# nghiahuynh-ai/Flamed-TTS

Hardware: AMD Instinct MI355X
Metric: latent frames/s (RTF at nsteps-denoiser=128) (higher is better)
Workload: dtype bf16; 1 GPU; BASELINE configs[1]: 1 utterance(s) x 400 frames (5.0 s audio) per GPU, nsteps-denoiser=128, bf16 (one persistent launch per solve); batch_per_gpu=1, frames=400, nfe=128, global_batch=1, parallelism=utterance-sharded x1 (no collectives)

## Files before the change

### flamed-tts_amd/csrc/capi.cpp

```cpp
#include <cstdarg>
#include <cstdio>
#include <cstring>
#include <mutex>

#include "common.hpp"
#include "flamed_hip.h"

namespace fl {
static thread_local char g_err[1024] = "";

void set_error(const char* fmt, ...) {
  va_list ap;
  va_start(ap, fmt);
  vsnprintf(g_err, sizeof(g_err), fmt, ap);
  va_end(ap);
}
const char* last_error() { return g_err; }

int device_of(const void* p, int* dev) {
  if (!p || !dev) return kBadArg;
  hipPointerAttribute_t a;
  if (hipPointerGetAttributes(&a, p) != hipSuccess) {
    (void)hipGetLastError();
    return kBadArg;
// ... 34 lines not shown
  static const int k_smax[] = {1, 2, 4, 0};
  static const Knob knobs[] = {
      {"splitk_target", &Tune::split_target, 1, 1 << 20, nullptr},
      {"splitk_max", &Tune::split_max, 1, 4, k_smax},
      {"small_stages", &Tune::small_stages, 3, 7, k_stages},
      {"xcd_strips", &Tune::xcd_strips, 0, 64, nullptr},
      {"bn32", &Tune::bn32, 0, 1, nullptr},
      {"dma", &Tune::use_dma, 0, 2, nullptr},
      {"dma_ns", &Tune::dma_ns, 3, 8, k_dmans},
      {"noctr", &Tune::noctr, 0, 1, nullptr},
      {"dup_class", &Tune::dup_class, -1, FLAMED_DEN_KERNEL_CLASSES - 1, nullptr},
      {"stamp_class", &Tune::stamp_class, -1, FLAMED_DEN_KERNEL_CLASSES - 1, nullptr},
      {"dw_cg32", &Tune::dw_cg32_rows, 0, 1 << 30, nullptr},
      {"dw_cg", &Tune::dw_cg_small, 16, 32, k_dwcg},
      {"dw_tc", &Tune::dw_tc_big, 64, 128, k_dwtc},
      {"big", &Tune::big, 0, 1, nullptr},
      {"big_rows", &Tune::big_min_rows, 1024, 1 << 30, nullptr},
      {"big_ns", &Tune::big_ns, 2, 3, k_bigns},
      {"lnfold", &Tune::lnfold, 0, 1, nullptr},
      {"fold_rows", &Tune::fold_big_rows, 0, 1 << 30, nullptr},
      {"graph_steps", &Tune::graph_steps, 1, 1024, nullptr},
      {"x16", &Tune::x16, 0, 1, nullptr},
      {"g8p_rows", &Tune::g8p_rows, 0, 1 << 30, nullptr},
      {"dwgn", &Tune::dwgn, 0, 1, nullptr},
      {"dwgn_small", &Tune::dwgn_small, 0, 1, nullptr},
      {"fuse_euler", &Tune::fuse_euler, 0, 1, nullptr},
      {"pva_split", &Tune::pva_split, 0, 1, nullptr},
      {"persist", &Tune::persist, 0, 1, nullptr},
      {"split_batch", &Tune::split_batch, 1, 4, nullptr},
      {"split_graph", &Tune::split_graph, 0, 1, nullptr},
      {"split_prio", &Tune::split_prio, 0, 2, nullptr},
      {"prio_all", &Tune::prio_all, 0, 1, nullptr},
      {"split_min_rows", &Tune::split_min_rows, 1024, 1 << 30, nullptr},
      {"persist_opt", &Tune::persist_opt, 0, (1 << 23) - 1, nullptr},
      {"persist_seal_skip", &Tune::persist_seal_skip, -1, 1 << 20, nullptr},
      {"persist_inject", &Tune::persist_inject, -1, 1 << 20, nullptr},
      {"persist_multi", &Tune::persist_multi, 0, 1, nullptr},
      {"persist_pad", &Tune::persist_pad, 0, 1, nullptr},
      {"persist_pad_ntw", &Tune::persist_pad_ntw, 1, 8, nullptr},
      {"persist_as", &Tune::persist_as, 0, 8, nullptr},
      {"persist_multi_ntw", &Tune::persist_multi_ntw, 1, 8, nullptr},
      {"persist_ntw", &Tune::persist_ntw, 1, 8, nullptr},
      {"persist_capmode", &Tune::persist_capmode, 0, 1, nullptr},
      {"pva_persist", &Tune::pva_persist, 0, 1, nullptr},
      {"attn_mfma", &Tune::attn_mfma, 0, 1, nullptr},
      {"prior_split", &Tune::prior_split, 0, 1, nullptr},
      {"enc_skip", &Tune::enc_skip, 0, 1, nullptr},
      {"stop_after", &Tune::stop_after, -1, 1 << 20, nullptr},
      {"coop", &Tune::coop, 0, 1, nullptr},
      {"dwgn_var", &Tune::dwgn_var, 0, 2, nullptr},
      {"pva_stage", &Tune::pva_stage, 0, 3, nullptr},
      {"pva_inject", &Tune::pva_inject, -1, 1 << 20, nullptr},
      {"adaln_grouped", &Tune::adaln_grouped, 0, 1, nullptr},
  };
  for (const Knob& k : knobs) {
    if (std::strcmp(k.name, key) != 0) continue;
    int v = value;
    if (k.lo == 0 && k.hi == 1) v = value != 0;
    FL_REQUIRE(v >= k.lo && v <= k.hi, "flamed_tune: %s must be in [%d, %d] (got %d)", key, k.lo, k.hi, value);
    if (k.allowed) {
      bool ok = false;
      for (const int* a = k.allowed; *a; ++a) ok = ok || *a == v;
      FL_REQUIRE(ok, "flamed_tune: %s = %d is not a supported value", key, value);
    }
    t.*(k.field) = v;
    return kOk;
  }
// ... 20 lines not shown
```

### flamed-tts_amd/csrc/persist.hip

```cpp
#include <cstdio>
#include <cstdlib>

#include "flamed_hip.h"
#include "flamed_diag.h"
#include "persist.hpp"
#include "gemm_dma.hpp"

namespace fl {
namespace pk {

#ifdef FL_STAMPS
constexpr int kStampSlots = 160;
#define PST(step)                                                                                       \
  do {                                                                                                  \
    if ((step) == P.pst_step && P.pst && threadIdx.x == 0 && pst_k < kStampSlots)                       \
      P.pst[blockIdx.x * kStampSlots + pst_k] = __builtin_amdgcn_s_memrealtime();                      \
    ++pst_k;                                                                                            \
  } while (0)
#define PSTP(step) \
  (((step) == P.pst_step && P.pst && pst_k < kStampSlots) ? P.pst + blockIdx.x * kStampSlots + pst_k++ : (++pst_k, nullptr))
#define GND(k, v)                                                                                       \
  do {                                                                                                  \
    if (cur_step == P.gnd_step && P.gnd)                                                                \
      P.gnd[(((size_t)blk * kWGs + g * kSlots + s) * 32 + (tid & 31)) * 32 + (k)] = (v);                \
// ... 152 lines not shown
}

template <int K, class RowB>
__device__ __forceinline__ void dma_panel4(char* dst, const void* base, RowB rowb, int wave, int lane_in, bool w4 = true) {
  constexpr int kRowB = 2 * K, kNI = 32 * kRowB / 1024;
  static_assert(kNI % 4 == 0, "pieces per wave");
  if (!w4 && wave == 0) return;
  const int w0 = w4 ? wave : wave - 1, ws = w4 ? 4 : 3;
  const int lane = opq(lane_in);
  const unsigned long long b = (unsigned long long)(uintptr_t)base;
  const unsigned blo = (unsigned)__builtin_amdgcn_readfirstlane((unsigned)b);
  const unsigned bhi = (unsigned)__builtin_amdgcn_readfirstlane((unsigned)(b >> 32));
  const unsigned long long bs = ((unsigned long long)bhi << 32) | (unsigned long long)blo;
  const unsigned l0 = __builtin_amdgcn_readfirstlane((unsigned)(uintptr_t)((__attribute__((address_space(3))) char*)(dst)));
#pragma unroll
  for (int j = 0; j < (kNI + 2) / 3; ++j) {
    const int i = w0 + ws * j;
    if (i >= kNI) break;
    const unsigned pos = (unsigned)i * 1024u + (unsigned)lane * 16u;
    const int n = (int)(pos / kRowB);
    const unsigned jl = (pos % kRowB) >> 4;
    const unsigned off = rowb(n) + ((jl ^ (unsigned)(n & 15)) << 4);
    const unsigned l = l0 + (unsigned)i * 1024u;
    unsigned keep;
    asm volatile("s_mov_b32 %0, m0\n\ts_mov_b32 m0, %3\n\ts_nop 0\n\tglobal_load_lds_dwordx4 %1, %2\n\ts_mov_b32 m0, %0"
                 : "=&s"(keep)
                 : "v"(off), "s"(bs), "s"(l)
                 : "memory");
  }
}

__device__ __forceinline__ unsigned frag_group_bytes(int KST) { return (unsigned)(4 * kMaxNTW * KST * 1024); }

template <int K>
__device__ __forceinline__ void gemm(const bf16* A, int r0, int nr, const char* wl, f32x4 (&acc)[2], int wave, int lane_in,
                                     unsigned long long* stamp = nullptr, int g = 0, bool frag = false, int tile = -1,
                                     bool first = true) {
  constexpr int KST = K / 32;
  const int lane = opq(lane_in);
  if (tile < 0) tile = wave;
  acc[0] = f32x4{0.f, 0.f, 0.f, 0.f};
  acc[1] = f32x4{0.f, 0.f, 0.f, 0.f};
  const int ntile = (nr + 15) >> 4;
  const int c = lane & 15, q = lane >> 4;
  u32x4 a[KST];
  if (tile < ntile) {
    if (frag) {
      const __amdgpu_buffer_rsrc_t rs =
          rsrc(reinterpret_cast<const char*>(A) + (size_t)g * frag_group_bytes(KST), frag_group_bytes(KST));
      const unsigned base = (unsigned)(((tile * KST) * 64 + lane) * 16);
#pragma unroll
      for (int ks = 0; ks < KST; ++ks) a[ks] = ld16(rs, base + ks * 1024);
    } else {
      const __amdgpu_buffer_rsrc_t rs = rsrc(A + (size_t)r0 * K, (unsigned)nr * K * 2);
      const unsigned base = (unsigned)(((16 * tile + c) * K + q * 8) * 2);
#pragma unroll
      for (int ks = 0; ks < KST; ++ks) a[ks] = ld16(rs, base + ks * 64);
    }
    if (first) asm volatile("s_waitcnt vmcnt(%0)" ::"i"(KST) : "memory");
    else asm volatile("s_waitcnt vmcnt(0)" ::: "memory");
  } else {
    asm volatile("s_waitcnt vmcnt(0)" ::: "memory");
  }
  if (first) __syncthreads();
  if (first && stamp && threadIdx.x == 0) *stamp = __builtin_amdgcn_s_memrealtime();
  if (tile < ntile) {
    constexpr int kBP = 4;
    u32x4 b0[kBP], b1[kBP];
#pragma unroll
    for (int p = 0; p < kBP; ++p) {
      b0[p] = *reinterpret_cast<const u32x4*>(wl + woff<K>(c, 4 * p + q));
      b1[p] = *reinterpret_cast<const u32x4*>(wl + woff<K>(16 + c, 4 * p + q));
    }
#pragma unroll
    for (int ks = 0; ks < KST; ++ks) {
      const u32x4 x0 = b0[ks % kBP], x1 = b1[ks % kBP];
      if (ks + kBP < KST) {
        b0[ks % kBP] = *reinterpret_cast<const u32x4*>(wl + woff<K>(c, 4 * (ks + kBP) + q));
        b1[ks % kBP] = *reinterpret_cast<const u32x4*>(wl + woff<K>(16 + c, 4 * (ks + kBP) + q));
      }
      acc[0] = __builtin_amdgcn_mfma_f32_16x16x32_bf16(__builtin_bit_cast(bf16x8, x0), __builtin_bit_cast(bf16x8, a[ks]), acc[0], 0, 0, 0);
      acc[1] = __builtin_amdgcn_mfma_f32_16x16x32_bf16(__builtin_bit_cast(bf16x8, x1), __builtin_bit_cast(bf16x8, a[ks]), acc[1], 0, 0, 0);
    }
  }
}

template <int K, int NTW>
__device__ __forceinline__ void gemm_multi(const bf16* A, int r0, int nr, const char* wl, f32x4 (&acc)[NTW][2], int wave,
                                           int lane_in, unsigned long long* stamp, int g, bool frag) {
  constexpr int KST = K / 32, KU = KST / 2, U = 2 * NTW;
  static_assert(KST % 2 == 0, "half-tile units");
  const int lane = opq(lane_in);
  const int ntile = (nr + 15) >> 4;
  const int c = lane & 15, q = lane >> 4;
  const __amdgpu_buffer_rsrc_t rs = frag ? rsrc(reinterpret_cast<const char*>(A) + (size_t)g * frag_group_bytes(KST), frag_group_bytes(KST))
                                         : rsrc(A + (size_t)r0 * K, (unsigned)nr * K * 2);
  u32x4 a[2][KU];
  auto load = [&](u32x4 (&dst)[KU], int u) __attribute__((always_inline)) {
    const int tile = wave + 4 * (u >> 1), k0 = (u & 1) * KU;
    if (tile >= ntile) return;
    if (frag) {
      const unsigned base = (unsigned)(((tile * KST + k0) * 64 + lane) * 16);
#pragma unroll
      for (int ks = 0; ks < KU; ++ks) dst[ks] = ld16(rs, base + ks * 1024);
    } else {
      const unsigned base = (unsigned)(((16 * tile + c) * K + k0 * 32 + q * 8) * 2);
#pragma unroll
      for (int ks = 0; ks < KU; ++ks) dst[ks] = ld16(rs, base + ks * 64);
    }
  };
  load(a[0], 0);
  if (wave < ntile) asm volatile("s_waitcnt vmcnt(%0)" ::"i"(KU) : "memory");
// ... 405 lines not shown

__device__ __forceinline__ float2 gn_finalize(const float (&nv)[kGroups], const float (&mv)[kGroups], const float (&qv)[kGroups],
                                              int utt, int gpu, int T, float gw) {
#pragma clang fp contract(off)
  float n = 0.f, mean = 0.f, m2 = 0.f;
#pragma unroll
  for (int k = 0; k < kGroups; ++k) {
    const bool mine = k / gpu == utt;
    chan_combine_rn(n, mean, m2, mine ? nv[k] : 0.f, mine ? mv[k] : 0.f, mine ? qv[k] : 0.f);
  }
  return make_float2(mean, (1.0f / sqrtf(m2 * (1.0f / (float)T) + 1e-5f)) * gw);
}

template <bool KH, int NTW, bool RK2 = false, bool RAG = false>
__global__ __launch_bounds__(kThreads, 1) void den_persist_kernel(Params P) {
  extern __shared__ __attribute__((aligned(16))) char smem[];
  const int tid = threadIdx.x, lane = tid & 63;
  const int wave = __builtin_amdgcn_readfirstlane(tid >> 6);
  const int T = P.T;
  const int TT = P.B * P.T;
  const int H = kH;
  int g = blockIdx.x % kGroups, s = blockIdx.x / kGroups;
  if (P.opt & 8) {
    const int x = g, j = s;
    g = 4 * (x / 4) + (j % 4);
    s = 8 * (x % 4) + j / 4;
  }
  constexpr bool xloc = false;
  const bool frag = (P.opt & 64) != 0;
  constexpr bool kDefer = NTW == 1 && !KH;
  const bool gran = (P.opt & 512) != 0;
  constexpr bool kTileMajor = true;
  const bool tm = kTileMajor && !(P.opt & 2097152);
  const int gpu = kGroups / P.B, utt = g / gpu;
  auto len_of = [&](int k) {
    if constexpr (RAG) return P.lens[k / gpu];
    else return T;
  };
  const int Tu = len_of(g);
  int r0, nr;
  group_rows(g, T, Tu, P.B, r0, nr, P.opt);
  const int ub = utt * T, ue = ub + Tu;
  const bool idle = P.Bx > 0 && utt >= P.Bx;
  const int MB = P.Bx > 0 ? P.Bx : P.B, mutt = idle ? P.Bx - 1 : utt;
  const int c = lane & 15, q = lane >> 4;
  const int col0 = kCols * s;
  char* stg = smem + L_HS;
  float* hs = reinterpret_cast<float*>(smem + L_HS);
  float* st = reinterpret_cast<float*>(smem + L_ST);
  float* red = reinterpret_cast<float*>(smem + L_RED);
  float4* gnv = reinterpret_cast<float4*>(smem + L_GNV);
  int* flag = reinterpret_cast<int*>(smem + L_FLAG);
  constexpr bool kOneWord = one_word_variant(KH, NTW, RK2, RAG);
  const ArriveImage ai = arrive_image(kOneWord ? kOptOneWord : P.opt, g, s);
  int* const grp = P.ctr + (kOneWord ? CT_GRP : ai.abase());
  int* const mygrp = kOneWord ? grp + 16 * g : P.ctr + ai.base;
  int* const mysig = kOneWord ? mygrp : P.ctr + ai.sig;
  const int gws = kOneWord ? 0 : ai.stride(), gwn = kOneWord ? 1 : ai.n();
  const int aws = kOneWord ? 16 : ai.stride(), awn = kOneWord ? kGroups : ai.an();
  auto gtarget = [&](int l) { return kOneWord ? 32 * l : ai.target(l); };
  int* gnc = P.ctr + CT_GN + 16 * s;
  int* errw = P.ctr + CT_ERR;
  int* fails = P.sticky + SY_FAILS;
  const long long tmo = P.tmo;
  int L = 0;
  int ndg = 0;
// ... 44 lines not shown
  const int xr_row = tid >> 2, xch = kCh * s + 2 * (tid & 3);
  float xs0[NTW], xs1[NTW];
#pragma unroll
  for (int i = 0; i < NTW; ++i) {
    xs0[i] = 0.f;
    xs1[i] = 0.f;
    const int row = kChunk * i + xr_row;
    if (row < nr && !idle) {
      xs0[i] = P.xt[(size_t)(r0 + row) * kC + xch];
      xs1[i] = P.xt[(size_t)(r0 + row) * kC + xch + 1];
    }
  }
  constexpr bool kStash = RK2 && NTW >= 3;
  [[maybe_unused]] float xb0[RK2 && !kStash ? NTW : 1], xb1[RK2 && !kStash ? NTW : 1];
  if constexpr (RK2 && !kStash) {
#pragma unroll
    for (int i = 0; i < NTW; ++i) {
      xb0[i] = xs0[i];
      xb1[i] = xs1[i];
    }
  }
  const bool seal = (P.opt & 16384) != 0;
  const bool dseal = (P.opt & 65536) != 0;
  int dseal_v = 0x7fffffff, dseal_tgt = 0;
  auto dseal_check = [&]() {
    if (dseal && wave == 0) {
      const bool ok = __all(dseal_v >= dseal_tgt);
      if (!ok && lane == 0) raise_err(errw, fails, 4);
      return ok;
    }
    return true;
  };
  auto seal_put = [&]() {
    dseal_check();
    if ((seal || dseal) && tid == 0 && !(cur_step == P.seal_skip && blockIdx.x == 5))
      __hip_atomic_store(P.seal + 4 * (g * kSlots + s), L + 1, __ATOMIC_RELAXED, __HIP_MEMORY_SCOPE_AGENT);
  };
  auto seal_wait = [&](int g0, int ng) -> bool {
    if (dseal) {
      if (wave == 0) {
        const int gi = ng == 1 ? g0 : (lane < 32 ? (g + kGroups - 1) % kGroups : (g + 1) % kGroups);
        dseal_v = __hip_atomic_load(P.seal + 4 * (gi * kSlots + (lane & 31)), __ATOMIC_RELAXED, __HIP_MEMORY_SCOPE_AGENT);
        dseal_tgt = L;
      }
      return true;
    }
    return !seal || seals_ok(P.seal + 4 * g0 * kSlots, ng * kSlots, L, P.ctr + CT_ERR, P.sticky + SY_FAILS, P.tmo,
                             reinterpret_cast<int*>(smem + L_FLAG));
  };
  auto fail_exit = [&]() {
#pragma unroll
    for (int i = 0; i < NTW; ++i) {
      const int row = kChunk * i + xr_row;
      if (row < nr && !idle) {
        P.xt[(size_t)(r0 + row) * kC + xch] = __builtin_nanf("");
        P.xt[(size_t)(r0 + row) * kC + xch + 1] = __builtin_nanf("");
      }
    }
  };
  const bool wlocal = (P.opt & 32768) != 0;
  auto stage_sync = [&]() {
    if (wlocal) asm volatile("s_waitcnt lgkmcnt(0)" ::: "memory");
    else __syncthreads();
  };
  dma_panel<kC>(smem, [&](int n) { return P.win + (size_t)(col0 + n) * kC; }, wave, lane, P.opt);
  auto publish_xs = [&]() {
    bf16* t = reinterpret_cast<bf16*>(stg);
#pragma unroll
    for (int i = 0; i < NTW; ++i) {
      const int nrc = crows(i);
      if (i > 0) stage_sync();
      t[xr_row * kCh + 2 * (tid & 3)] = (bf16)xs0[i];
      t[xr_row * kCh + 2 * (tid & 3) + 1] = (bf16)xs1[i];
      stage_sync();
      const int prow = 16 * wave + lane;
      if (frag) {
        if (lane < 16 && 16 * wave < nrc) {
          const __amdgpu_buffer_rsrc_t rs =
              rsrc(reinterpret_cast<char*>(P.xs) + (size_t)g * frag_group_bytes(kC / 32), frag_group_bytes(kC / 32));
          const int tt = 4 * i + wave, ln = lane + 16 * (s & 3);
          const u32x4 v = prow < nrc ? *reinterpret_cast<const u32x4*>(stg + prow * 16) : u32x4{0u, 0u, 0u, 0u};
          const unsigned off = (unsigned)(((tt * (kC / 32) + (s >> 2)) * 64 + ln) * 16);
          if (xloc) st16p(rs, off, v);
          else st16(rs, off, v);
        }
      } else if (lane < 16 && prow < nrc) {
        const __amdgpu_buffer_rsrc_t rs = rsrc(P.xs, (unsigned)TT * kC * 2);
        const unsigned off = (unsigned)(((size_t)(r0 + kChunk * i + prow) * kC + kCh * s) * 2);
        if (xloc) st16p(rs, off, *reinterpret_cast<const u32x4*>(stg + prow * 16));
        else st16(rs, off, *reinterpret_cast<const u32x4*>(stg + prow * 16));
      }
    }
    seal_put();
    signal(mysig);
    ++L;
  };
  {
    unsigned* const a0 = reinterpret_cast<unsigned*>(P.sticky + SY_ARRIVE0);
    unsigned* const a1 = reinterpret_cast<unsigned*>(P.sticky + SY_ARRIVE1);
    unsigned* tk = reinterpret_cast<unsigned*>(smem + L_FLAG);
    if (tid == 0) tk[1] = __hip_atomic_fetch_add(a0, 1u, __ATOMIC_RELAXED, __HIP_MEMORY_SCOPE_AGENT);
    __syncthreads();
    const unsigned target = arrive_target(tk[1]);
    __syncthreads();
    const bool ok0 = arrive_wait(a0, target, tmo, flag);
    if (ok0) {
      constexpr int kRst = kOneWord ? 4 : kResetInts, kRstN = kOneWord ? kCtrOneInts : kCtrInts;
      if (tid < kRst && kRstN > kRst * (int)blockIdx.x + tid)
        __hip_atomic_store(P.ctr + kRst * blockIdx.x + tid, 0, __ATOMIC_RELAXED, __HIP_MEMORY_SCOPE_AGENT);
      if (tid < 4) __hip_atomic_store(P.seal + 4 * blockIdx.x + tid, 0, __ATOMIC_RELAXED, __HIP_MEMORY_SCOPE_AGENT);
      if (gran && tid < 32) {
        const __amdgpu_buffer_rsrc_t rq = rsrc(P.gnp, kGroups * kH * 16);
        st16(rq, (unsigned)((blockIdx.x * 32 + tid) * 16), u32x4{0u, 0u, 0u, 0u});
      }
      if (tid < 8) {
        const __amdgpu_buffer_rsrc_t ry = rsrc(P.yb, kWGs * 2 * kCh * 8);
        st16(ry, (unsigned)((blockIdx.x * 8 + tid) * 16), u32x4{0u, 0u, 0u, 0u});
      }
      asm volatile("s_waitcnt vmcnt(0)" ::: "memory");
    }
    __syncthreads();
    if (tid == 0) __hip_atomic_fetch_add(a1, 1u, __ATOMIC_RELAXED, __HIP_MEMORY_SCOPE_AGENT);
    const bool ok1 = arrive_wait(a1, target, tmo, flag);
    if (!ok0 || !ok1) {
      if (tid == 0) {
        unsigned* pf = reinterpret_cast<unsigned*>(P.sticky + SY_PFAIL);
        if (__hip_atomic_exchange(pf, target, __ATOMIC_RELAXED, __HIP_MEMORY_SCOPE_AGENT) != target)
// ... 59 lines not shown
    float binv[2][4];
    ld_cols(binv, P.bin + col0, q);
    PST(step);
    if (!wait_ge<!kOneWord>(errw, fails, tmo, mygrp, gws, gwn, gtarget(L), flag) || !seal_wait(g, 1)) { fail_exit(); return; }
    PST(step);
    f32x4 accm[NTW][2];
    if constexpr (KH) gemm_kh<kC>(P.xs, r0, nr, (smem + wb * kWPanel), accm[0], wave, lane, PSTP(step), g, frag);
    else if constexpr (NTW == 1) gemm<kC>(P.xs, r0, nr, (smem + wb * kWPanel), accm[0], wave, lane, PSTP(step), g, frag);
    else gemm_chunks<kC, NTW>(P.xs, r0, nr, (smem + wb * kWPanel), accm, wave, lane, PSTP(step), g, frag, P.opt);
    PST(step);
#pragma unroll
    for (int ci = 0; ci < NTW; ++ci) {
      const int tl = wave + 4 * ci;
      const f32x4(&acc)[2] = accm[ci];
      acc_to(X[ci], acc);
#pragma unroll
      for (int nt = 0; nt < 2; ++nt)
#pragma unroll
        for (int i = 0; i < 4; ++i) X[ci][nt][i] += binv[nt][i];
      if (16 * tl < nr) {
        store_partials_t(P.xpart[0], X[ci], r0, nr, s, tl, lane, g, tm);
        store_halo_t(P.ximg, X[ci], r0, nr, col0, tl, TT, lane);
      }
    }
    seal_put();
    if (dmafirst) {
      next_w(P.blk[0].w2);
      signal_dma<16>(mysig);
    } else {
      signal(mysig);
      next_w(P.blk[0].w2);
    }
    PST(step);
    ++L;

    for (int blk = 0; blk <= P.NB; ++blk) {
      const bool fin = blk == P.NB;
      const BlockW& bw = P.blk[blk];
      const float* mb = md + (size_t)blk * 6 * H;

      const int cc = tid & 31, rg = tid >> 5;
      float hsc[4], hsh[4], hlw[4], hlb[4], osc[2][4], osh[2][4], olw[2][4], olb[2][4];
      constexpr bool kWide = NTW <= 4;
      if constexpr (!kWide) {
#pragma unroll
        for (int e = 0; e < 4; ++e) {
          const int col = col0 + 4 * (tid & 7) + e;
          hsc[e] = mb[H + col];
          hsh[e] = mb[col];
          hlw[e] = fin ? 1.0f : bw.lnw[col];
          hlb[e] = fin ? 0.0f : bw.lnb[col];
        }
      } else {
        const int col = col0 + 4 * (tid & 7);
        const float4 a = *reinterpret_cast<const float4*>(mb + H + col), b = *reinterpret_cast<const float4*>(mb + col);
        hsc[0] = a.x; hsc[1] = a.y; hsc[2] = a.z; hsc[3] = a.w;
        hsh[0] = b.x; hsh[1] = b.y; hsh[2] = b.z; hsh[3] = b.w;
        float4 lw = make_float4(1.0f, 1.0f, 1.0f, 1.0f), lb = make_float4(0.0f, 0.0f, 0.0f, 0.0f);
        if (!fin) {
          lw = *reinterpret_cast<const float4*>(bw.lnw + col);
          lb = *reinterpret_cast<const float4*>(bw.lnb + col);
        }
        hlw[0] = lw.x; hlw[1] = lw.y; hlw[2] = lw.z; hlw[3] = lw.w;
        hlb[0] = lb.x; hlb[1] = lb.y; hlb[2] = lb.z; hlb[3] = lb.w;
      }
      ld_cols(osc, mb + H + col0, q);
// ... 91 lines not shown
          }
        }
        __syncthreads();
        if (ci == 0) PST(step);
        {
          float win[8 + kTaps - 1];
#pragma unroll
          for (int j = 0; j < 8 + kTaps - 1; ++j) win[j] = hs[(8 * rg + j) * kHsLd + cc];
#pragma unroll
          for (int k = 0; k < 8; ++k) {
            float a = dbias;
#pragma unroll
            for (int j = 0; j < kTaps; ++j) a = fmaf(w[j], win[k + j], a);
            d[ci][k] = a;
          }
        }
      }
      PST(step);
      {
        float sm = 0.f;
#pragma unroll
        for (int ci = 0; ci < NTW; ++ci) {
          const int nv = min(max(crows(ci) - 8 * rg, 0), 8);
#pragma unroll
          for (int k = 0; k < 8; ++k)
            if (k < nv) sm += d[ci][k];
        }
        red[rg * kCols + cc] = sm;
        __syncthreads();
        float tot = 0.f;
#pragma unroll
        for (int k = 0; k < 8; ++k) tot += red[k * kCols + cc];
        const float mg = nr > 0 ? tot / (float)nr : 0.f;
        __syncthreads();
        float m2 = 0.f;
#pragma unroll
        for (int ci = 0; ci < NTW; ++ci) {
          const int nv = min(max(crows(ci) - 8 * rg, 0), 8);
#pragma unroll
          for (int k = 0; k < 8; ++k)
            if (k < nv) {
              const float e = d[ci][k] - mg;
              m2 = fmaf(e, e, m2);
            }
        }
        red[rg * kCols + cc] = m2;
        __syncthreads();
        if (tid < kCols) {
          float m2t = 0.f;
#pragma unroll
          for (int k = 0; k < 8; ++k) m2t += red[k * kCols + cc];
          GND(26, mg);
          GND(27, m2t);
          GND(28, (float)nr);
          if (gran) {
            unsigned long long* gq = reinterpret_cast<unsigned long long*>(P.gnp) + ((size_t)g * H + col0 + cc) * 2;
            const unsigned long long tag = (unsigned long long)(ndg + 1) << 32;
            __hip_atomic_store(gq, tag | __float_as_uint(mg), __ATOMIC_RELAXED, __HIP_MEMORY_SCOPE_AGENT);
            __hip_atomic_store(gq + 1, tag | __float_as_uint(m2t), __ATOMIC_RELAXED, __HIP_MEMORY_SCOPE_AGENT);
          } else {
            const __amdgpu_buffer_rsrc_t rq = rsrc(P.gnp, kGroups * kH * 16);
            st16(rq, (unsigned)((g * H + col0 + cc) * 16), __builtin_bit_cast(u32x4, make_float4((float)nr, mg, m2t, 0.f)));
          }
        }
      }
      if (!gran) signal(gnc);
      PST(step);
      ++ndg;
      PST(step);
      if (gran) {
        bool ok = true;
        if (tid < 64) {
          const unsigned long long* gq = reinterpret_cast<const unsigned long long*>(P.gnp) + (size_t)(col0 + (tid & 31)) * 2;
          float mv[kGroups], qv[kGroups];
          const unsigned long long t0 = __builtin_amdgcn_s_memrealtime();
          for (unsigned it = 0;; ++it) {
            bool mine = true;
            if (tid < kCols) {
#pragma unroll
              for (int k = 0; k < kGroups; ++k) {
                const unsigned long long a = __hip_atomic_load(gq + (size_t)k * H * 2, __ATOMIC_RELAXED, __HIP_MEMORY_SCOPE_AGENT);
                const unsigned long long b = __hip_atomic_load(gq + (size_t)k * H * 2 + 1, __ATOMIC_RELAXED, __HIP_MEMORY_SCOPE_AGENT);
                mine = mine && (unsigned)(a >> 32) == (unsigned)ndg && (unsigned)(b >> 32) == (unsigned)ndg;
                mv[k] = __uint_as_float((unsigned)a);
// ... 43 lines not shown
#pragma unroll
        for (int k = 0; k < kGroups; ++k) {
          const float4 v = as_f4(ld16(rq, (unsigned)((k * H + col0 + tid) * 16)));
          nv[k] = v.x;
          mv[k] = v.y;
          qv[k] = v.z;
          GND(3 * k, v.x);
          GND(3 * k + 1, v.y);
          GND(3 * k + 2, v.z);
        }
        const float2 ms = gn_finalize(nv, mv, qv, utt, gpu, Tu, gwv);
        GND(24, ms.x);
        GND(25, ms.y);
        gnv[tid] = make_float4(ms.x, ms.y, gbv, 0.f);
      }
      }
      __syncthreads();
      {
        const float4 gv = gnv[cc];
        bf16* t = reinterpret_cast<bf16*>(stg);
#pragma unroll
        for (int ci = 0; ci < NTW; ++ci) {
          if (ci > 0) stage_sync();
#pragma unroll
          for (int k = 0; k < 8; ++k) t[(8 * rg + k) * kCols + cc] = (bf16)((d[ci][k] - gv.x) * gv.y + gv.z);
          stage_sync();
          if (frag) flush_frag(stg, P.a2, g, s, crows(ci), kH / 32, xloc, 4 * ci);
          else flush_tile<bf16>(stg, P.a2, H, r0 + kChunk * ci, 0, crows(ci), col0, TT, xloc);
        }
      }
      seal_put();
      signal(mysig);
      PST(step);
      ++L;

      float b2v[2][4];
      ld_cols(b2v, bw.b2 + col0, q);
      PST(step);
      if (!wait_ge<!kOneWord>(errw, fails, tmo, mygrp, gws, gwn, gtarget(L), flag) || !seal_wait(g, 1)) { fail_exit(); return; }
      PST(step);
      f32x4 accm_c2[NTW][2];
      if constexpr (KH) gemm_kh<kH>(P.a2, r0, nr, (smem + wb * kWPanel), accm_c2[0], wave, lane, PSTP(step), g, frag);
      else if constexpr (NTW == 1) gemm<kH>(P.a2, r0, nr, (smem + wb * kWPanel), accm_c2[0], wave, lane, PSTP(step), g, frag);
      else gemm_chunks<kH, NTW>(P.a2, r0, nr, (smem + wb * kWPanel), accm_c2, wave, lane, PSTP(step), g, frag, P.opt);
      PST(step);
#pragma unroll
      for (int ci = 0; ci < NTW; ++ci) {
        const int tl = wave + 4 * ci;
        const f32x4(&acc)[2] = accm_c2[ci];
        float v[2][4];
#pragma unroll
        for (int nt = 0; nt < 2; ++nt) {
#pragma unroll
          for (int i = 0; i < 4; ++i) v[nt][i] = gelu_fast(acc[nt][i] + b2v[nt][i]);
        }
        if (16 * tl < nr) store_op_t(P.u, g, s, tl, v, r0, nr, col0, TT, lane, frag);
        if (ci == 0) PST(step);
      }
      seal_put();
      if (dmafirst) {
        next_w(bw.w3);
        signal_dma<16>(mysig);
      } else {
#ifdef FL_STAMPS
        asm volatile("s_waitcnt vmcnt(0)" ::: "memory");
        PST(step);
        __syncthreads();
        PST(step);
#endif
        signal(mysig);
        next_w(bw.w3);
      }
      PST(step);
      ++L;

      float g3[2][4], b3v[2][4], alv[2][4], alw[2][4];
      ld_cols(g3, mb + 2 * H + col0, q);
      ld_cols(b3v, bw.b3 + col0, q);
      ld_cols(alv, mb + 4 * H + col0, q);
      if (fin) fill_cols(alw, 1.0f);
      else ld_cols(alw, bw.lnmw + col0, q);
      PST(step);
      if (!wait_ge<!kOneWord>(errw, fails, tmo, mygrp, gws, gwn, gtarget(L), flag) || !seal_wait(g, 1)) { fail_exit(); return; }
      PST(step);
#pragma unroll
      for (int nt = 0; nt < 2; ++nt)
#pragma unroll
        for (int r = 0; r < 4; ++r) alv[nt][r] = fin ? 1.0f + alv[nt][r] : alw[nt][r] * (1.0f + alv[nt][r]);
      f32x4 accm_c3[NTW][2];
      if constexpr (KH) gemm_kh<kH>(P.u, r0, nr, (smem + wb * kWPanel), accm_c3[0], wave, lane, PSTP(step), g, frag);
      else if constexpr (NTW == 1) gemm<kH>(P.u, r0, nr, (smem + wb * kWPanel), accm_c3[0], wave, lane, PSTP(step), g, frag);
      else gemm_chunks<kH, NTW>(P.u, r0, nr, (smem + wb * kWPanel), accm_c3, wave, lane, PSTP(step), g, frag, P.opt);
      PST(step);
#pragma unroll
      for (int ci = 0; ci < NTW; ++ci) {
        const int tl = wave + 4 * ci;
        const f32x4(&acc)[2] = accm_c3[ci];
        float v[2][4];
        const int p = 16 * tl + c + kHalo;
        const float mean = st[2 * p], rstd = st[2 * p + 1];
#pragma unroll
        for (int nt = 0; nt < 2; ++nt) {
#pragma unroll
          for (int i = 0; i < 4; ++i) {
            const float xh = (X[ci][nt][i] - mean) * rstd;
            const float h = xh * ova[nt][i] + ovb[nt][i];
            X[ci][nt][i] = X[ci][nt][i] + g3[nt][i] * (h + (acc[nt][i] + b3v[nt][i]));
            v[nt][i] = X[ci][nt][i] * alv[nt][i];
          }
        }
        if (16 * tl < nr) {
          store_partials_t(P.xpart[1], X[ci], r0, nr, s, tl, lane, g, tm);
          store_op_t(P.xa, g, s, tl, v, r0, nr, col0, TT, lane, frag);
        }
      }
      seal_put();
      if (dmafirst) {
        if (fin) issue_out();
        else next_w(bw.m0);
        signal_dma<16>(mysig);
      } else {
        signal(mysig);
        if (fin) issue_out();
        else next_w(bw.m0);
      }
      PST(step);
      ++L;
      if (fin) break;

      const float* fo0 = md + P.MS0 + (size_t)blk * 2 * H;
      float fa0[2][4], fb0[2][4];
      ld_cols(fa0, fo0 + col0, q);
      ld_cols(fb0, fo0 + H + col0, q);
      PST(step);
      if (!wait_ge<!kOneWord>(errw, fails, tmo, mygrp, gws, gwn, gtarget(L), flag) || !seal_wait(g, 1)) { fail_exit(); return; }
      PST(step);
      [[maybe_unused]] u32x4 rp_m0[8];
      if constexpr (kDefer) load_row_partials(rp_m0, P.xpart[1], TT, r0, nr, wave, lane, g, tm);
      else row_stats(P.xpart[1], TT, r0, r0 + nr, r0 - kHalo, st, tm, own_base);
      f32x4 accm_m0[NTW][2];
      if constexpr (KH) gemm_kh<kH>(P.xa, r0, nr, (smem + wb * kWPanel), accm_m0[0], wave, lane, PSTP(step), g, frag);
      else if constexpr (NTW == 1) gemm<kH>(P.xa, r0, nr, (smem + wb * kWPanel), accm_m0[0], wave, lane, PSTP(step), g, frag);
      else gemm_chunks<kH, NTW>(P.xa, r0, nr, (smem + wb * kWPanel), accm_m0, wave, lane, PSTP(step), g, frag, P.opt);
      PST(step);
#pragma unroll
      for (int ci = 0; ci < NTW; ++ci) {
        const int tl = wave + 4 * ci;
        const f32x4(&acc)[2] = accm_m0[ci];
        float v[2][4];
        float mean, rstd;
        if constexpr (kDefer) {
          const float2 ms = finish_row_partials(rp_m0, lane);
          mean = ms.x;
          rstd = ms.y;
        } else {
          const int p = 16 * tl + c + kHalo;
          mean = st[2 * p];
          rstd = st[2 * p + 1];
        }
#pragma unroll
        for (int nt = 0; nt < 2; ++nt) {
#pragma unroll
          for (int i = 0; i < 4; ++i) v[nt][i] = silu(rstd * (acc[nt][i] - mean * fa0[nt][i]) + fb0[nt][i]);
        }
        if (16 * tl < nr) store_op_t(P.u, g, s, tl, v, r0, nr, col0, TT, lane, frag);
      }
      seal_put();
      if (dmafirst) {
        next_w(bw.m2);
        signal_dma<16>(mysig);
      } else {
        signal(mysig);
        next_w(bw.m2);
      }
      PST(step);
      ++L;

      float g2v[2][4], bm2[2][4];
      ld_cols(g2v, mb + 5 * H + col0, q);
      ld_cols(bm2, bw.mb2 + col0, q);
      PST(step);
      if (!wait_ge<!kOneWord>(errw, fails, tmo, mygrp, gws, gwn, gtarget(L), flag) || !seal_wait(g, 1)) { fail_exit(); return; }
      PST(step);
      f32x4 accm_m2[NTW][2];
      if constexpr (KH) gemm_kh<kH>(P.u, r0, nr, (smem + wb * kWPanel), accm_m2[0], wave, lane, PSTP(step), g, frag);
      else if constexpr (NTW == 1) gemm<kH>(P.u, r0, nr, (smem + wb * kWPanel), accm_m2[0], wave, lane, PSTP(step), g, frag);
      else gemm_chunks<kH, NTW>(P.u, r0, nr, (smem + wb * kWPanel), accm_m2, wave, lane, PSTP(step), g, frag, P.opt);
      PST(step);
#pragma unroll
      for (int ci = 0; ci < NTW; ++ci) {
        const int tl = wave + 4 * ci;
        const f32x4(&acc)[2] = accm_m2[ci];
#pragma unroll
        for (int nt = 0; nt < 2; ++nt)
#pragma unroll
          for (int i = 0; i < 4; ++i) X[ci][nt][i] = X[ci][nt][i] + g2v[nt][i] * (acc[nt][i] + bm2[nt][i]);
        if (16 * tl < nr) {
          store_partials_t(P.xpart[0], X[ci], r0, nr, s, tl, lane, g, tm);
          store_halo_t(P.ximg, X[ci], r0, nr, col0, tl, TT, lane);
        }
      }
      seal_put();
      if (dmafirst) {
        next_w(P.blk[blk + 1].w2);
        signal_dma<16>(mysig);
      } else {
        signal(mysig);
        next_w(P.blk[blk + 1].w2);
      }
      PST(step);
      ++L;
    }

    wb ^= 1;
    float fac[2][4], fbc[2][4];
    {
      const float* fo = md + P.MS0 + (size_t)P.NB * 2 * H;
#pragma unroll
      for (int nt = 0; nt < 2; ++nt) {
        const int n = 16 * nt + 4 * q, m = n < 24 ? n : n - 24;
        const int ns = (m >> 3) * kC + kCh * s + (m & 7);
        const float4 a = *reinterpret_cast<const float4*>(fo + ns), b = *reinterpret_cast<const float4*>(fo + 3 * kC + ns);
        fac[nt][0] = a.x; fac[nt][1] = a.y; fac[nt][2] = a.z; fac[nt][3] = a.w;
        fbc[nt][0] = b.x; fbc[nt][1] = b.y; fbc[nt][2] = b.z; fbc[nt][3] = b.w;
      }
    }
    PST(step);
    if (!wait_ge<!kOneWord>(errw, fails, tmo, mygrp, gws, gwn, gtarget(L), flag) || !seal_wait(g, 1)) { fail_exit(); return; }
    PST(step);
    [[maybe_unused]] u32x4 rp_out[8];
    if constexpr (kDefer) load_row_partials(rp_out, P.xpart[1], TT, r0, nr, wave, lane, g, tm);
    else row_stats(P.xpart[1], TT, r0, r0 + nr, r0 - kHalo, st, tm, own_base);
    f32x4 acco[NTW][2];
    if constexpr (KH) gemm_kh<kH>(P.xa, r0, nr, (smem + wb * kWPanel), acco[0], wave, lane, PSTP(step), g, frag);
    else if constexpr (NTW == 1) gemm<kH>(P.xa, r0, nr, (smem + wb * kWPanel), acco[0], wave, lane, PSTP(step), g, frag);
    else gemm_chunks<kH, NTW>(P.xa, r0, nr, (smem + wb * kWPanel), acco, wave, lane, PSTP(step), g, frag, P.opt);
    PST(step);
    float* yl = reinterpret_cast<float*>(NTW == 1 ? stg : smem + wb * kWPanel);
    if (NTW > 1) __syncthreads();
#pragma unroll
    for (int ci = 0; ci < NTW; ++ci) {
      const int row = 16 * (wave + 4 * ci) + c, p = row + kHalo;
      if (NTW == 1 || row < nr) {
        float mean, rstd;
        if constexpr (kDefer) {
          const float2 ms = finish_row_partials(rp_out, lane);
          mean = ms.x;
          rstd = ms.y;
        } else {
          mean = st[2 * p];
          rstd = st[2 * p + 1];
        }
#pragma unroll
        for (int nt = 0; nt < 2; ++nt) {
          const int n0 = 16 * nt + 4 * q;
          if (n0 < 24) {
            float y[4];
#pragma unroll
            for (int i = 0; i < 4; ++i) y[i] = rstd * (acco[ci][nt][i] - mean * fac[nt][i]) + fbc[nt][i];
            *reinterpret_cast<float4*>(yl + row * 24 + n0) = make_float4(y[0], y[1], y[2], y[3]);
          }
        }
      }
    }
    __syncthreads();
    const unsigned ytag = (unsigned)(step - P.s0 + 1);
    if (tid < 2 * kCh && nr > 0 && !idle) {
      const float y = tid < kCh ? yl[(nr - 1) * 24 + tid] : yl[16 + tid - kCh];
      __hip_atomic_store(ybq + (size_t)(g + kGroups * s) * (2 * kCh) + tid, ((unsigned long long)ytag << 32) | __float_as_uint(y),
// ... 261 lines not shown
```

### flamed-tts_amd/csrc/persist.hpp

```cpp
#pragma once
#include "common.hpp"

namespace fl {
namespace pk {

constexpr int kGroups = 8, kSlots = 32, kWGs = kGroups * kSlots, kThreads = 256;
constexpr int kH = 1024, kC = 256, kCols = kH / kSlots, kCh = kC / kSlots;
constexpr int kChunk = 64, kMaxNTW = 8, kMaxRows = kChunk * kMaxNTW, kHalo = 15, kTaps = 31, kWin = kChunk + 2 * kHalo;
constexpr int kMaxNB = 8, kMaxT = kGroups * kMaxRows;
constexpr int kWPanel = kCols * kH * 2;
constexpr int kHsLd = kCols + 4;
constexpr int L_HS = 2 * kWPanel;
constexpr int L_ST = L_HS + kWin * kHsLd * 4;
constexpr int L_RED = L_ST + (kMaxRows + 2 * kHalo) * 8;
constexpr int L_GNV = L_RED + 8 * kCols * 4;
constexpr int L_FLAG = L_GNV + kCols * 16;
constexpr int kLds = (L_FLAG + 16 + 15) / 16 * 16;
static_assert(kLds <= 160 * 1024, "persistent solve LDS");
constexpr int kLineInts = 32, kShards = 4, kShardSlots = kSlots / kShards;
constexpr int CT_GRP = 0, CT_GN = 16 * kGroups, CT_ERR = CT_GN + 16 * kSlots, kCtrOneInts = CT_ERR + 16;
constexpr int CT_SHD = (kCtrOneInts + kLineInts - 1) / kLineInts * kLineInts;
constexpr int kCtrInts = CT_SHD + kGroups * kShards * kLineInts, kResetInts = 8;
static_assert(kCtrInts <= kWGs * kResetInts && kCtrOneInts <= kWGs * 4, "the reset prologue covers the block");
static_assert(CT_GN % kLineInts == 0 && CT_ERR % kLineInts == 0 && CT_ERR + kLineInts <= CT_SHD,
              "group words, GroupNorm words and the error word share no line");
constexpr int kOptOneWord = 1 << 22;
__host__ __device__ constexpr bool one_word_variant(bool KH, int NTW, bool RK2, bool RAG) {
  if (KH) return false;
  if (!RAG) return !RK2 ? (NTW == 4 || NTW == 5) : (NTW == 5 || NTW == 8);
  return !RK2 ? ((NTW >= 3 && NTW <= 5) || NTW == 7) : (NTW <= 3 || NTW == 5);
}
struct ArriveImage {
  int sig, base, sh;
  __host__ __device__ int n() const { return 1 << sh; }
  __host__ __device__ int an() const { return kGroups << sh; }
  __host__ __device__ int abase() const { return sh ? CT_SHD : CT_GRP; }
  __host__ __device__ int stride() const { return 16 << (sh >> 1); }
  __host__ __device__ int target(int L) const { return (kSlots * L) >> sh; }
};
static_assert((1 << 2) == kShards && (16 << 1) == kLineInts && (kSlots >> 2) == kShardSlots, "ArriveImage shifts");
__host__ __device__ inline ArriveImage arrive_image(int opt, int g, int s) {
  if (opt & kOptOneWord) return {CT_GRP + 16 * g, CT_GRP + 16 * g, 0};
  const int w = CT_SHD + g * kShards * kLineInts;
  return {w + (s / kShardSlots) * kLineInts, w, 2};
}
constexpr int SY_FAILS = 0, SY_ARRIVE0 = 32, SY_ARRIVE1 = 64, SY_PFAIL = 96, kStickyInts = 128;

__host__ __device__ inline unsigned arrive_target(unsigned ticket) {
  return ticket - ticket % (unsigned)kWGs + (unsigned)kWGs;
}
__host__ __device__ inline bool arrive_reached(unsigned cur, unsigned target) { return (int)(cur - target) >= 0; }

constexpr int kGroupTiles = kMaxRows / 16;
constexpr unsigned kXpartBytes = (unsigned)kGroups * kGroupTiles * kSlots * 128u;
static_assert(kXpartBytes >= (unsigned)kMaxT * kSlots * 8u, "row partial buffers");
__host__ __device__ inline unsigned xpart_off(int g, int lrow, int s) {
  return (unsigned)((((g * kGroupTiles + (lrow >> 4)) * kSlots + s) * 16 + (lrow & 15)) * 8);
}
__host__ __device__ inline void row_owner(int i, int Lu, int gpu, int opt, int& gi, int& lrow) {
// ... 68 lines not shown
```

Measured before the change: 23360 latent frames/s.

## Overlap row-partial loads and seal checks with the persistent-kernel GEMM

For the front variants (NTW<=2, non-KH), the row-partial loads for the next LayerNorm are issued inside the GEMM after the A-fragment loads, and the vmcnt wait is adjusted to cover them. The partial reduction can also be finished mid-GEMM through a scheduled callback. The second GroupNorm reduction gets its own LDS buffer so one __syncthreads can be dropped. The downstream seal check moves after the signal, and partial stores are reordered after the operand stores, so the critical-path stores go out first. New opt bits re-enable the old ordering; the default path changes for those variants at the cost of more LDS and more complex waitcnt reasoning.

Result: slower. 22810 latent frames/s (-2.3%).

```diff
diff --git a/flamed-tts_amd/csrc/capi.cpp b/flamed-tts_amd/csrc/capi.cpp
--- a/flamed-tts_amd/csrc/capi.cpp
+++ b/flamed-tts_amd/csrc/capi.cpp
@@ -90,7 +90,7 @@
       {"split_prio", &Tune::split_prio, 0, 2, nullptr},
       {"prio_all", &Tune::prio_all, 0, 1, nullptr},
       {"split_min_rows", &Tune::split_min_rows, 1024, 1 << 30, nullptr},
-      {"persist_opt", &Tune::persist_opt, 0, (1 << 23) - 1, nullptr},
+      {"persist_opt", &Tune::persist_opt, 0, (1 << 26) - 1, nullptr},
       {"persist_seal_skip", &Tune::persist_seal_skip, -1, 1 << 20, nullptr},
       {"persist_inject", &Tune::persist_inject, -1, 1 << 20, nullptr},
       {"persist_multi", &Tune::persist_multi, 0, 1, nullptr},
diff --git a/flamed-tts_amd/csrc/persist.hip b/flamed-tts_amd/csrc/persist.hip
--- a/flamed-tts_amd/csrc/persist.hip
+++ b/flamed-tts_amd/csrc/persist.hip
@@ -208,11 +208,16 @@
 
 __device__ __forceinline__ unsigned frag_group_bytes(int KST) { return (unsigned)(4 * kMaxNTW * KST * 1024); }
 
-template <int K>
+struct NoOp {
+  __device__ __forceinline__ void operator()() const {}
+};
+constexpr int kMidSteps = 8;
+template <int K, class Tail = NoOp, class Mid = NoOp>
 __device__ __forceinline__ void gemm(const bf16* A, int r0, int nr, const char* wl, f32x4 (&acc)[2], int wave, int lane_in,
                                      unsigned long long* stamp = nullptr, int g = 0, bool frag = false, int tile = -1,
-                                     bool first = true) {
+                                     bool first = true, int tailn = 0, Tail tail = Tail(), Mid mid = Mid()) {
   constexpr int KST = K / 32;
+  static_assert(KST + 16 <= 63, "vmcnt is a 6-bit count");
   const int lane = opq(lane_in);
   if (tile < 0) tile = wave;
   acc[0] = f32x4{0.f, 0.f, 0.f, 0.f};
@@ -233,9 +238,12 @@
 #pragma unroll
       for (int ks = 0; ks < KST; ++ks) a[ks] = ld16(rs, base + ks * 64);
     }
-    if (first) asm volatile("s_waitcnt vmcnt(%0)" ::"i"(KST) : "memory");
-    else asm volatile("s_waitcnt vmcnt(0)" ::: "memory");
+    tail();
+    if (!first) asm volatile("s_waitcnt vmcnt(0)" ::: "memory");
+    else if (tailn == 16) asm volatile("s_waitcnt vmcnt(%0)" ::"i"(KST + 16) : "memory");
+    else asm volatile("s_waitcnt vmcnt(%0)" ::"i"(KST) : "memory");
   } else {
+    tail();
     asm volatile("s_waitcnt vmcnt(0)" ::: "memory");
   }
   if (first) __syncthreads();
@@ -254,6 +262,10 @@
       if (ks + kBP < KST) {
         b0[ks % kBP] = *reinterpret_cast<const u32x4*>(wl + woff<K>(c, 4 * (ks + kBP) + q));
         b1[ks % kBP] = *reinterpret_cast<const u32x4*>(wl + woff<K>(16 + c, 4 * (ks + kBP) + q));
+      }
+      if (KST > kMidSteps && ks == KST - kMidSteps) {
+        if constexpr (!__is_same(Mid, NoOp)) __builtin_amdgcn_sched_barrier(0);
+        mid();
       }
       acc[0] = __builtin_amdgcn_mfma_f32_16x16x32_bf16(__builtin_bit_cast(bf16x8, x0), __builtin_bit_cast(bf16x8, a[ks]), acc[0], 0, 0, 0);
       acc[1] = __builtin_amdgcn_mfma_f32_16x16x32_bf16(__builtin_bit_cast(bf16x8, x1), __builtin_bit_cast(bf16x8, a[ks]), acc[1], 0, 0, 0);
@@ -725,6 +737,10 @@
   const bool gran = (P.opt & 512) != 0;
   constexpr bool kTileMajor = true;
   const bool tm = kTileMajor && !(P.opt & 2097152);
+  constexpr bool kFront = front_variant(KH, NTW, RK2, RAG);
+  [[maybe_unused]] const bool pfirst = !kFront || !tm || !frag || (P.opt & kOptPartialsFirst) != 0;
+  [[maybe_unused]] const bool onered = !kFront || (P.opt & kOptOneRed) != 0;
+  [[maybe_unused]] const bool epar = !kFront || (P.opt & kOptParentEpilogue) != 0;
   const int gpu = kGroups / P.B, utt = g / gpu;
   auto len_of = [&](int k) {
     if constexpr (RAG) return P.lens[k / gpu];
@@ -835,9 +851,13 @@
     return true;
   };
   auto seal_put = [&]() {
-    dseal_check();
+    if (epar) dseal_check();
     if ((seal || dseal) && tid == 0 && !(cur_step == P.seal_skip && blockIdx.x == 5))
       __hip_atomic_store(P.seal + 4 * (g * kSlots + s), L + 1, __ATOMIC_RELAXED, __HIP_MEMORY_SCOPE_AGENT);
+  };
+  auto seal_late = [&]() {
+    if constexpr (kFront)
+      if (!epar) dseal_check();
   };
   auto seal_wait = [&](int g0, int ng) -> bool {
     if (dseal) {
@@ -896,6 +916,7 @@
     }
     seal_put();
     signal(mysig);
+    seal_late();
     ++L;
   };
   {
@@ -1021,6 +1042,7 @@
       next_w(P.blk[0].w2);
     }
     PST(step);
+    seal_late();
     ++L;
 
     for (int blk = 0; blk <= P.NB; ++blk) {
@@ -1178,7 +1200,8 @@
 #pragma unroll
         for (int k = 0; k < 8; ++k) tot += red[k * kCols + cc];
         const float mg = nr > 0 ? tot / (float)nr : 0.f;
-        __syncthreads();
+        float* const red2 = onered ? red : reinterpret_cast<float*>(smem + L_RED2);
+        if (onered) __syncthreads();
         float m2 = 0.f;
 #pragma unroll
         for (int ci = 0; ci < NTW; ++ci) {
@@ -1190,12 +1213,12 @@
               m2 = fmaf(e, e, m2);
             }
         }
-        red[rg * kCols + cc] = m2;
+        red2[rg * kCols + cc] = m2;
         __syncthreads();
         if (tid < kCols) {
           float m2t = 0.f;
 #pragma unroll
-          for (int k = 0; k < 8; ++k) m2t += red[k * kCols + cc];
+          for (int k = 0; k < 8; ++k) m2t += red2[k * kCols + cc];
           GND(26, mg);
           GND(27, m2t);
           GND(28, (float)nr);
@@ -1305,6 +1328,7 @@
       seal_put();
       signal(mysig);
       PST(step);
+      seal_late();
       ++L;
 
       float b2v[2][4];
@@ -1345,6 +1369,7 @@
         next_w(bw.w3);
       }
       PST(step);
+      seal_late();
       ++L;
 
       float g3[2][4], b3v[2][4], alv[2][4], alw[2][4];
@@ -1383,8 +1408,9 @@
           }
         }
         if (16 * tl < nr) {
-          store_partials_t(P.xpart[1], X[ci], r0, nr, s, tl, lane, g, tm);
+          if (epar) store_partials_t(P.xpart[1], X[ci], r0, nr, s, tl, lane, g, tm);
           store_op_t(P.xa, g, s, tl, v, r0, nr, col0, TT, lane, frag);
+          if (!epar) store_partials_t(P.xpart[1], X[ci], r0, nr, s, tl, lane, g, tm);
         }
       }
       seal_put();
@@ -1398,6 +1424,7 @@
         else next_w(bw.m0);
       }
       PST(step);
+      seal_late();
       ++L;
       if (fin) break;
 
@@ -1409,12 +1436,26 @@
       if (!wait_ge<!kOneWord>(errw, fails, tmo, mygrp, gws, gwn, gtarget(L), flag) || !seal_wait(g, 1)) { fail_exit(); return; }
       PST(step);
       [[maybe_unused]] u32x4 rp_m0[8];
-      if constexpr (kDefer) load_row_partials(rp_m0, P.xpart[1], TT, r0, nr, wave, lane, g, tm);
-      else row_stats(P.xpart[1], TT, r0, r0 + nr, r0 - kHalo, st, tm, own_base);
+      [[maybe_unused]] float2 ms_m0 = make_float2(0.f, 0.f);
+      [[maybe_unused]] auto ldp_m0 = [&]() __attribute__((always_inline)) { load_row_partials(rp_m0, P.xpart[1], TT, r0, nr, wave, lane, g, tm); };
+      [[maybe_unused]] auto ldt_m0 = [&]() __attribute__((always_inline)) { load_row_partials(rp_m0, P.xpart[1], TT, r0, nr, wave, lane, g, true); };
+      [[maybe_unused]] auto fin_m0 = [&]() __attribute__((always_inline)) { ms_m0 = finish_row_partials(rp_m0, lane); };
+      if constexpr (!kDefer) row_stats(P.xpart[1], TT, r0, r0 + nr, r0 - kHalo, st, tm, own_base);
       f32x4 accm_m0[NTW][2];
       if constexpr (KH) gemm_kh<kH>(P.xa, r0, nr, (smem + wb * kWPanel), accm_m0[0], wave, lane, PSTP(step), g, frag);
-      else if constexpr (NTW == 1) gemm<kH>(P.xa, r0, nr, (smem + wb * kWPanel), accm_m0[0], wave, lane, PSTP(step), g, frag);
-      else gemm_chunks<kH, NTW>(P.xa, r0, nr, (smem + wb * kWPanel), accm_m0, wave, lane, PSTP(step), g, frag, P.opt);
+      else if constexpr (NTW == 1) {
+        unsigned long long* const stp = PSTP(step);
+        if (pfirst) {
+          ldp_m0();
+          gemm<kH>(P.xa, r0, nr, (smem + wb * kWPanel), accm_m0[0], wave, lane, stp, g, frag);
+          fin_m0();
+        } else if (epar) {
+          gemm<kH>(P.xa, r0, nr, (smem + wb * kWPanel), accm_m0[0], wave, lane, stp, g, true, -1, true, 16, ldt_m0);
+          fin_m0();
+        } else {
+          gemm<kH>(P.xa, r0, nr, (smem + wb * kWPanel), accm_m0[0], wave, lane, stp, g, true, -1, true, 16, ldt_m0, fin_m0);
+        }
+      } else gemm_chunks<kH, NTW>(P.xa, r0, nr, (smem + wb * kWPanel), accm_m0, wave, lane, PSTP(step), g, frag, P.opt);
       PST(step);
 #pragma unroll
       for (int ci = 0; ci < NTW; ++ci) {
@@ -1423,9 +1464,8 @@
         float v[2][4];
         float mean, rstd;
         if constexpr (kDefer) {
-          const float2 ms = finish_row_partials(rp_m0, lane);
-          mean = ms.x;
-          rstd = ms.y;
+          mean = ms_m0.x;
+          rstd = ms_m0.y;
         } else {
           const int p = 16 * tl + c + kHalo;
           mean = st[2 * p];
@@ -1447,6 +1487,7 @@
         next_w(bw.m2);
       }
       PST(step);
+      seal_late();
       ++L;
 
       float g2v[2][4], bm2[2][4];
@@ -1469,8 +1510,9 @@
 #pragma unroll
           for (int i = 0; i < 4; ++i) X[ci][nt][i] = X[ci][nt][i] + g2v[nt][i] * (acc[nt][i] + bm2[nt][i]);
         if (16 * tl < nr) {
-          store_partials_t(P.xpart[0], X[ci], r0, nr, s, tl, lane, g, tm);
+          if (epar) store_partials_t(P.xpart[0], X[ci], r0, nr, s, tl, lane, g, tm);
           store_halo_t(P.ximg, X[ci], r0, nr, col0, tl, TT, lane);
+          if (!epar) store_partials_t(P.xpart[0], X[ci], r0, nr, s, tl, lane, g, tm);
         }
       }
       seal_put();
@@ -1482,6 +1524,7 @@
         next_w(P.blk[blk + 1].w2);
       }
       PST(step);
+      seal_late();
       ++L;
     }
 
@@ -1502,12 +1545,20 @@
     if (!wait_ge<!kOneWord>(errw, fails, tmo, mygrp, gws, gwn, gtarget(L), flag) || !seal_wait(g, 1)) { fail_exit(); return; }
     PST(step);
     [[maybe_unused]] u32x4 rp_out[8];
-    if constexpr (kDefer) load_row_partials(rp_out, P.xpart[1], TT, r0, nr, wave, lane, g, tm);
-    else row_stats(P.xpart[1], TT, r0, r0 + nr, r0 - kHalo, st, tm, own_base);
+    [[maybe_unused]] auto ldp_out = [&]() __attribute__((always_inline)) { load_row_partials(rp_out, P.xpart[1], TT, r0, nr, wave, lane, g, tm); };
+    [[maybe_unused]] auto ldt_out = [&]() __attribute__((always_inline)) { load_row_partials(rp_out, P.xpart[1], TT, r0, nr, wave, lane, g, true); };
+    if constexpr (!kDefer) row_stats(P.xpart[1], TT, r0, r0 + nr, r0 - kHalo, st, tm, own_base);
     f32x4 acco[NTW][2];
     if constexpr (KH) gemm_kh<kH>(P.xa, r0, nr, (smem + wb * kWPanel), acco[0], wave, lane, PSTP(step), g, frag);
-    else if constexpr (NTW == 1) gemm<kH>(P.xa, r0, nr, (smem + wb * kWPanel), acco[0], wave, lane, PSTP(step), g, frag);
-    else gemm_chunks<kH, NTW>(P.xa, r0, nr, (smem + wb * kWPanel), acco, wave, lane, PSTP(step), g, frag, P.opt);
+    else if constexpr (NTW == 1) {
+      unsigned long long* const stp = PSTP(step);
+      if (pfirst) {
+        ldp_out();
+        gemm<kH>(P.xa, r0, nr, (smem + wb * kWPanel), acco[0], wave, lane, stp, g, frag);
+      } else {
+        gemm<kH>(P.xa, r0, nr, (smem + wb * kWPanel), acco[0], wave, lane, stp, g, true, -1, true, 16, ldt_out);
+      }
+    } else gemm_chunks<kH, NTW>(P.xa, r0, nr, (smem + wb * kWPanel), acco, wave, lane, PSTP(step), g, frag, P.opt);
     PST(step);
     float* yl = reinterpret_cast<float*>(NTW == 1 ? stg : smem + wb * kWPanel);
     if (NTW > 1) __syncthreads();
diff --git a/flamed-tts_amd/csrc/persist.hpp b/flamed-tts_amd/csrc/persist.hpp
--- a/flamed-tts_amd/csrc/persist.hpp
+++ b/flamed-tts_amd/csrc/persist.hpp
@@ -15,8 +15,10 @@
 constexpr int L_RED = L_ST + (kMaxRows + 2 * kHalo) * 8;
 constexpr int L_GNV = L_RED + 8 * kCols * 4;
 constexpr int L_FLAG = L_GNV + kCols * 16;
-constexpr int kLds = (L_FLAG + 16 + 15) / 16 * 16;
+constexpr int L_RED2 = (L_FLAG + 16 + 15) / 16 * 16;
+constexpr int kLds = L_RED2 + 8 * kCols * 4;
 static_assert(kLds <= 160 * 1024, "persistent solve LDS");
+static_assert(L_ST >= L_HS + kWin * kHsLd * 4 && L_RED2 >= L_FLAG + 16, "the window / staging tile and the flag end below what follows them");
 constexpr int kLineInts = 32, kShards = 4, kShardSlots = kSlots / kShards;
 constexpr int CT_GRP = 0, CT_GN = 16 * kGroups, CT_ERR = CT_GN + 16 * kSlots, kCtrOneInts = CT_ERR + 16;
 constexpr int CT_SHD = (kCtrOneInts + kLineInts - 1) / kLineInts * kLineInts;
@@ -25,6 +27,11 @@
 static_assert(CT_GN % kLineInts == 0 && CT_ERR % kLineInts == 0 && CT_ERR + kLineInts <= CT_SHD,
               "group words, GroupNorm words and the error word share no line");
 constexpr int kOptOneWord = 1 << 22;
+constexpr int kOptPartialsFirst = 1 << 23, kOptOneRed = 1 << 24, kOptParentEpilogue = 1 << 25;
+__host__ __device__ constexpr bool front_variant(bool KH, int NTW, bool RK2, bool RAG) {
+  if (KH || NTW > 2) return false;
+  return !RAG || (NTW == 2 && !RK2);
+}
 __host__ __device__ constexpr bool one_word_variant(bool KH, int NTW, bool RK2, bool RAG) {
   if (KH) return false;
   if (!RAG) return !RK2 ? (NTW == 4 || NTW == 5) : (NTW == 5 || NTW == 8);
```
